# Farama-Foundation/HighwayEnv

Measured on NVIDIA H100. Metric: env-steps/sec (batched), highway-fast-v0 50 veh, higher is better.
Workload: dtype f64

## Files before the change

highwayenv_b200/csrc/hwy_highway.cu:

```cuda
#include <cstdio>
#include <cstdlib>
#include <cstring>
#include <algorithm>
#include <atomic>
#include <cstddef>
#include <mutex>

#include <cuda_runtime.h>

#include "../../include/hwyb200.h"
#include "hwy_device.cuh"
#include "hwy_math.cuh"

namespace hwy {

#ifdef HWY_PHASE_TIMING
__device__ unsigned long long g_phase_cycles[16];
#define PHASE_INIT() long long _pt = clock64()
#define PHASE_MARK(k)                                                                 \
    do {                                                                              \
        long long _n = clock64();                                                     \
        if ((threadIdx.x & 31) == 0) atomicAdd(&g_phase_cycles[k], (unsigned long long)(_n - _pt)); \
        _pt = _n;                                                                     \
    } while (0)
#else
#define PHASE_INIT()
#define PHASE_MARK(k)
#endif

template <int TPE>
struct Frame {
    static constexpr int NW = TPE / 32;
    double x[TPE], y[TPE], c[TPE], s[TPE], v[TPE], ts[TPE];
    double ls[TPE];
    __align__(16) float lsf[TPE];
    uint32_t smask[HWY_MAX_LANES][NW];
    uint32_t tm[HWY_MAX_LANES][NW];
    uint32_t lane_is[HWY_MAX_LANES][NW];
    uint32_t fired[NW];
    unsigned char lane[TPE], tgt[TPE], perm[TPE], rank[TPE];
    int slow;
    unsigned vmax_bits;
};

template <int TPE>
struct EnvShared {
    static constexpr int NW = TPE / 32;
    Frame<TPE> f[2];
    double key[TPE];
    uint32_t geo[TPE][NW];
    uint32_t mid[NW];
    uint32_t ok_left[NW], ok_right[NW];
    int n_items;
    unsigned short items[2 * TPE];
    double free_t[TPE], acc_own[TPE], delta[TPE];
    signed char f_own[TPE], r_own[TPE];
    uint32_t ctrl[NW], cc[NW];
    int last_will[TPE];
    unsigned char crash_hit[TPE];
    double sp_x[TPE];
    int done, sp_fallback;
};

template <int TPE>
__device__ __forceinline__ void env_sync() {
    __syncthreads();
}
template <int TPE, int LEVEL>
__device__ __forceinline__ void env_sync_phase() {
    __syncthreads();
}

template <int NW>
__device__ __forceinline__ bool test_bit(const uint32_t (&m)[NW], int i) {
    return (m[i >> 5] >> (i & 31)) & 1u;
}

__device__ __forceinline__ int lane_id() {
    int l;
    asm volatile("mov.u32 %0, %%laneid;" : "=r"(l));
    return l;
}

__device__ __forceinline__ void segment_or(uint32_t* words, uint32_t ballot, int i, int V) {
    const int lane = lane_id();
    if (i >= V || (i != 0 && lane != 0)) return;
    const int n = min(V - i, 32 - lane);
    const uint32_t m = (ballot >> lane) & (0xffffffffu >> (32 - n));
    if (!m) return;
    const int sh = i & 31;
    atomicOr(&words[i >> 5], m << sh);
    const uint32_t hi = __funnelshift_l(m, 0u, sh);
    if (hi) atomicOr(&words[(i >> 5) + 1], hi);
}
__device__ __forceinline__ uint32_t segment_leads(int i, bool active, int& mine) {
    const int lane = lane_id();
    const uint32_t lead = __ballot_sync(0xffffffffu, active && (i == 0 || lane == 0));
    mine = __popc(lead & (0xffffffffu >> (31 - lane))) - 1;
    return lead;
}

template <int TPE>
__device__ __noinline__ void neighbours_linear(const Frame<TPE>& F, const HwyStraightLane L, int V,
                                               int self, int& front, int& rear) {
    double s = lane_s(L, F.x[self], F.y[self]);
    double s_front = 0, s_rear = 0;
    front = -1;
    rear = -1;
    for (int v = 0; v < V; ++v) {
        if (v == self) continue;
        double s_v, lat_v;
        lane_local(L, F.x[v], F.y[v], s_v, lat_v);
        if (!lane_on(L, s_v, lat_v, 1.0)) continue;
        if (s <= s_v && (front < 0 || s_v <= s_front)) {
            s_front = s_v;
            front = v;
        }
        if (s_v < s && (rear < 0 || s_v > s_rear)) {
            s_rear = s_v;
            rear = v;
        }
    }
}

template <int TPE>
__device__ __forceinline__ void neighbours(const HwyHighwayParams& P, const Frame<TPE>& F, int V, int l,
                                           int self, int& front, int& rear) {
    constexpr int NW = TPE / 32;
    if (F.slow) {
        neighbours_linear(F, P.lanes[l], V, self, front, rear);
        return;
    }
    const int r = F.rank[self];
    const int w0 = r >> 5, b = r & 31;
    front = -1;
    rear = -1;
    uint32_t m = F.smask[l][w0] & (b == 31 ? 0u : (~0u << (b + 1)));
    int w = w0;
    while (m == 0 && ++w < NW) m = F.smask[l][w];
    if (m) front = F.perm[w * 32 + __ffs(m) - 1];
    m = F.smask[l][w0] & ((1u << b) - 1u);
    w = w0;
    while (m == 0 && --w >= 0) m = F.smask[l][w];
    if (m) rear = F.perm[w * 32 + 31 - __clz(m)];
}

template <int TPE>
__device__ __noinline__ int neighbours_packed(const uint32_t* __restrict__ smask_l, const Frame<TPE>& F, int self) {
    constexpr int NW = TPE / 32;
    const int r = F.rank[self];
    const int w0 = r >> 5, b = r & 31;
    int front = 0xff, rear = 0xff;
    uint32_t m = smask_l[w0] & (b == 31 ? 0u : (~0u << (b + 1)));
    int w = w0;
    while (m == 0 && ++w < NW) m = smask_l[w];
    if (m) front = F.perm[w * 32 + __ffs(m) - 1];
    m = smask_l[w0] & ((1u << b) - 1u);
    w = w0;
    while (m == 0 && --w >= 0) m = smask_l[w];
    if (m) rear = F.perm[w * 32 + 31 - __clz(m)];
    return front | (rear << 8);
}
template <int TPE>
__device__ __forceinline__ void neighbours_cold(const HwyHighwayParams& P, const Frame<TPE>& F, int V, int l,
                                                int self, int& front, int& rear) {
    if (F.slow) {
        neighbours_linear(F, P.lanes[l], V, self, front, rear);
        return;
    }
    const int fr = neighbours_packed(F.smask[l], F, self);
    front = (fr & 0xff) == 0xff ? -1 : (fr & 0xff);
    rear = (fr >> 8) == 0xff ? -1 : (fr >> 8);
}

struct IdmK {
    double comfort_acc_max, distance_wanted, time_wanted, two_sqrt_ab;
};
__device__ __forceinline__ IdmK make_idm(const HwyHighwayParams& P) {
    IdmK k;
    k.comfort_acc_max = P.comfort_acc_max;
    k.distance_wanted = P.distance_wanted;
    k.time_wanted = P.time_wanted;
    k.two_sqrt_ab = 2 * sqrt(-P.comfort_acc_max * P.comfort_acc_min);
    return k;
}
template <int TPE>
__device__ __forceinline__ double desired_gap(const IdmK& K, const Frame<TPE>& F, int ego, int front) {
    double dvx = F.v[ego] * F.c[ego] - F.v[front] * F.c[front];
    double dvy = F.v[ego] * F.s[ego] - F.v[front] * F.s[front];
    double dv = dot2(dvx, dvy, F.c[ego], F.s[ego]);
    return K.distance_wanted + F.v[ego] * K.time_wanted + F.v[ego] * dv / K.two_sqrt_ab;
}
template <int TPE>
__device__ __forceinline__ double lane_distance(const HwyHighwayParams& P, const Frame<TPE>& F,
                                                bool aligned, int ego, int other) {
// ... 186 lines not shown
                if (obs_env2) obs_env2[NF * pad + col] = 0.0f;
            }
        }
    } else if (i < K && i >= filled) {
        for (int col = 0; col < NF; ++col) {
            obs_env[NF * i + col] = 0.0f;
            if (obs_env2) obs_env2[NF * i + col] = 0.0f;
        }
    }
}

struct VehicleRegs {
    double x, y, heading, speed, target_speed, timer, delta, imp_x, imp_y;
    int meta;
};

__device__ __forceinline__ void load_vehicle(const HwyHighwayState& S, size_t slot, VehicleRegs& r) {
    double2 a = reinterpret_cast<const double2*>(S.pos)[slot];
    double2 b = reinterpret_cast<const double2*>(S.hs)[slot];
    double2 c = reinterpret_cast<const double2*>(S.tt)[slot];
    double2 d = reinterpret_cast<const double2*>(S.imp)[slot];
    r.x = a.x;
    r.y = a.y;
    r.heading = b.x;
    r.speed = b.y;
    r.target_speed = c.x;
    r.timer = c.y;
    r.imp_x = d.x;
    r.imp_y = d.y;
    r.delta = S.delta[slot];
    r.meta = S.meta[slot];
}
__device__ __forceinline__ void store_vehicle(const HwyHighwayState& S, size_t slot,
                                              const VehicleRegs& r) {
    reinterpret_cast<double2*>(S.pos)[slot] = make_double2(r.x, r.y);
    reinterpret_cast<double2*>(S.hs)[slot] = make_double2(r.heading, r.speed);
    reinterpret_cast<double2*>(S.tt)[slot] = make_double2(r.target_speed, r.timer);
    reinterpret_cast<double2*>(S.imp)[slot] = make_double2(r.imp_x, r.imp_y);
    S.meta[slot] = r.meta;
}

template <int TPE, bool LINEAR = false, bool DENSE = false>
__device__ __forceinline__ void publish(const HwyHighwayParams& P, Frame<TPE>& F, int i, bool active,
                                        const VehicleRegs& r) {
    constexpr int NW = TPE / 32;
    if (active) {
        double sn, cs;
        m_sincos(r.heading, &sn, &cs);
        F.x[i] = r.x;
        F.y[i] = r.y;
        F.c[i] = cs;
        F.s[i] = sn;
        F.v[i] = r.speed;
        F.ts[i] = meta_kind(r.meta) == HWY_KIND_VEHICLE ? (LINEAR ? r.speed : 0.0) : r.target_speed;
        F.ls[i] = lane_s(P.lanes[0], r.x, r.y);
        F.lsf[i] = (float)F.ls[i];
        F.lane[i] = (unsigned char)meta_lane(r.meta);
        F.tgt[i] = (unsigned char)meta_target(r.meta);
    }
    if (!DENSE && i < HWY_MAX_LANES * NW) (&F.smask[0][0])[i] = 0;
    if (i == 0) {
        F.slow = 0;
        F.vmax_bits = 0u;
    }
}

template <int TPE>
__device__ __forceinline__ void clear_masks(Frame<TPE>& F, int i, int V) {
    constexpr int kWords = (3 * HWY_MAX_LANES + 1) * (TPE / 32);
    static_assert(offsetof(Frame<TPE>, fired) + sizeof(F.fired) - offsetof(Frame<TPE>, smask) == 4 * kWords,
                  "mask words of Frame are not adjacent");
#pragma unroll 1
    for (int k = i; k < kWords; k += V) (&F.smask[0][0])[k] = 0;
}

template <int TPE>
__device__ __forceinline__ bool pair_precheck(const Frame<TPE>& F, int a, int b, double dt) {
    const double diag = sqrt(kVehLength * kVehLength + kVehWidth * kVehWidth);
    const double thr = (diag + diag) / 2 + F.v[a] * dt;
    const double dx = F.x[b] - F.x[a], dy = F.y[b] - F.y[a];
    return !(thr >= 0.0 && dx * dx + dy * dy > thr * thr * 1.000001 + 1e-9);
}
template <int TPE>
__device__ __noinline__ void pair_sat(const Frame<TPE>& F, int a, int b, double dt, bool& inter,
                                      bool& will, double& trx, double& try_) {
    {
        const double diag = sqrt(kVehLength * kVehLength + kVehWidth * kVehWidth);
        const double thr = (diag + diag) / 2 + F.v[a] * dt;
        const double dist = norm2(F.x[b] - F.x[a], F.y[b] - F.y[a]);
        if (dist > thr) {
            inter = false;
            will = false;
            trx = try_ = 0.0;
            return;
        }
    }
    {
        const double hl = kVehLength / 2, hw = kVehWidth / 2, margin = 1e-6;
        const double ca = F.c[a], sa = F.s[a], cb = F.c[b], sb = F.s[b];
        const double dx = F.x[b] - F.x[a], dy = F.y[b] - F.y[a];
        const double rvx = (F.v[a] * ca - F.v[b] * cb) * dt, rvy = (F.v[a] * sa - F.v[b] * sb) * dt;
        const double cd = fabs(ca * cb + sa * sb), sd = fabs(sa * cb - ca * sb);
        bool separated = false;
        separated |= fabs(dx * ca + dy * sa) - (hl + hl * cd + hw * sd) - fabs(rvx * ca + rvy * sa) > margin;
        separated |= fabs(-dx * sa + dy * ca) - (hw + hl * sd + hw * cd) - fabs(-rvx * sa + rvy * ca) > margin;
        separated |= fabs(dx * cb + dy * sb) - (hl + hl * cd + hw * sd) - fabs(rvx * cb + rvy * sb) > margin;
        separated |= fabs(-dx * sb + dy * cb) - (hw + hl * sd + hw * cd) - fabs(-rvx * sb + rvy * cb) > margin;
        if (separated) {
            inter = false;
            will = false;
            trx = try_ = 0.0;
            return;
        }
    }
    Quad pa = make_polygon(F.x[a], F.y[a], F.c[a], F.s[a]);
    Quad pb = make_polygon(F.x[b], F.y[b], F.c[b], F.s[b]);
    polygons_intersecting(pa, pb, F.v[a] * F.c[a] * dt, F.v[a] * F.s[a] * dt, F.v[b] * F.c[b] * dt,
                          F.v[b] * F.s[b] * dt, inter, will, trx, try_);
}

template <int TPE>
__device__ __noinline__ int rank_count(const Frame<TPE>& F, int V, int i, bool active) {
    const double si = active ? F.ls[i] : 0.0;
    const float fi = active ? F.lsf[i] : 0.0f;
    int rank = 0;
    bool ambiguous = false;
    const float4* lsf4 = reinterpret_cast<const float4*>(F.lsf);
    const int n4 = V >> 2;
    for (int q = 0; q < n4; ++q) {
        float4 f = lsf4[q];
        const int u = q << 2;
        rank += (f.x < fi) + (f.y < fi) + (f.z < fi) + (f.w < fi);
        ambiguous = ambiguous || (f.x == fi && u != i) || (f.y == fi && u + 1 != i) ||
                    (f.z == fi && u + 2 != i) || (f.w == fi && u + 3 != i);
    }
    for (int u = n4 << 2; u < V; ++u) {
        float fu = F.lsf[u];
        rank += fu < fi;
        ambiguous = ambiguous || (fu == fi && u != i);
    }
    bool tie = false;
    if (ambiguous) {
        rank = 0;
#pragma unroll 1
        for (int u = 0; u < V; ++u) {
            double su = F.ls[u];
            rank += (su < si) || (su == si && u < i);
            tie = tie || (su == si && u != i);
        }
    }
    return rank | ((int)tie << 8);
}

template <int TPE, bool DENSE>
__device__ __noinline__ int rank_repair(const Frame<TPE>& F, const Frame<TPE>& prev, int V, int i, bool active) {
    constexpr int NW = TPE / 32;
    uint32_t inv[NW];
    uint32_t bad = 0;
    if constexpr (!DENSE) {
        const int wl = i & 31;
#pragma unroll
        for (int w = 0; w < NW; ++w) {
            const int k = w * 32 + wl + 1;
            const bool in = k < V;
            const float a = in ? F.lsf[prev.perm[k - 1]] : 0.0f, c = in ? F.lsf[prev.perm[k]] : 1.0f;
            bool wrong = in && !(a < c) && !(a > c);
            if (in && a > c) {
                if (k >= 2 && !(F.lsf[prev.perm[k - 2]] < c)) wrong = true;
                if (k + 1 < V && !(a < F.lsf[prev.perm[k + 1]])) wrong = true;
            }
            inv[w] = __ballot_sync(0xffffffffu, in && a > c);
            bad |= __ballot_sync(0xffffffffu, wrong);
        }
    } else {
        const int lane = lane_id();
        int mine;
        int s = 0;
        for (uint32_t lead = segment_leads(i, active, mine); lead; lead &= lead - 1, ++s) {
            const ptrdiff_t d = (ptrdiff_t)(s - mine) * (ptrdiff_t)sizeof(EnvShared<TPE>);
            const Frame<TPE>& Fs = *reinterpret_cast<const Frame<TPE>*>(reinterpret_cast<const char*>(&F) + d);
            const Frame<TPE>& Ps = *reinterpret_cast<const Frame<TPE>*>(reinterpret_cast<const char*>(&prev) + d);
            uint32_t s_inv[NW];
            uint32_t s_bad = 0;
#pragma unroll
            for (int w = 0; w < NW; ++w) {
                const int k = w * 32 + lane + 1;
                const bool in = k < V;
                const float a = in ? Fs.lsf[Ps.perm[k - 1]] : 0.0f, c = in ? Fs.lsf[Ps.perm[k]] : 1.0f;
                bool wrong = in && !(a < c) && !(a > c);
                if (in && a > c) {
                    if (k >= 2 && !(Fs.lsf[Ps.perm[k - 2]] < c)) wrong = true;
                    if (k + 1 < V && !(a < Fs.lsf[Ps.perm[k + 1]])) wrong = true;
                }
                s_inv[w] = __ballot_sync(0xffffffffu, in && a > c);
                s_bad |= __ballot_sync(0xffffffffu, wrong);
            }
            if (s == mine) {
#pragma unroll
                for (int w = 0; w < NW; ++w) inv[w] = s_inv[w];
                bad = s_bad;
            }
        }
    }
#pragma unroll
    for (int w = 0; w < NW; ++w) {
        uint32_t near = (inv[w] << 1) | (inv[w] << 2);
        if (w > 0) near |= (inv[w - 1] >> 31) | (inv[w - 1] >> 30);
        bad |= inv[w] & near;
    }
    if (bad) return -1;
    if (!active) return 0;
    const int r0 = prev.rank[i];
    uint32_t w_dn = 0, w_up = 0;
#pragma unroll
    for (int w = 0; w < NW; ++w) {
        if (r0 >= 1 && w == ((r0 - 1) >> 5)) w_dn = inv[w];
        if (w == (r0 >> 5)) w_up = inv[w];
    }
    if (r0 >= 1 && ((w_dn >> ((r0 - 1) & 31)) & 1u)) return r0 - 1;
    if (r0 + 1 < V && ((w_up >> (r0 & 31)) & 1u)) return r0 + 1;
    return r0;
}

template <int TPE, bool DENSE>
__device__ __forceinline__ void build_frame(const HwyHighwayParams& P, EnvShared<TPE>& sm, Frame<TPE>& F,
                                            int i, bool active, bool aligned, const VehicleRegs& r,
                                            double dt, bool do_sweep, bool pruned, const Frame<TPE>* prev) {
    const int V = P.n_vehicles;
    const int wie = i >> 5;
    const int lane = meta_lane(r.meta), tgt = meta_target(r.meta);
    int rank = 0;
    bool reuse = false;
    if (prev && !DENSE) {
        bool ok = true;
#pragma unroll 1
        for (int k = (i & 31) + 1; k < V; k += 32) ok = ok && (F.lsf[prev->perm[k - 1]] < F.lsf[prev->perm[k]]);
        reuse = __all_sync(0xffffffffu, ok);
    } else if (prev) {
        int mine, s = 0;
#pragma unroll 1
        for (uint32_t lead = segment_leads(i, active, mine); lead; lead &= lead - 1, ++s) {
            const ptrdiff_t d = (ptrdiff_t)(s - mine) * (ptrdiff_t)sizeof(EnvShared<TPE>);
            const Frame<TPE>& Fs = *reinterpret_cast<const Frame<TPE>*>(reinterpret_cast<const char*>(&F) + d);
            const Frame<TPE>& Ps = *reinterpret_cast<const Frame<TPE>*>(reinterpret_cast<const char*>(prev) + d);
            bool ok = true;
#pragma unroll 1
            for (int k = lane_id() + 1; k < V; k += 32)
                ok = ok && (Fs.lsf[Ps.perm[k - 1]] < Fs.lsf[Ps.perm[k]]);
            ok = __all_sync(0xffffffffu, ok);
            if (s == mine) reuse = ok;
        }
    }
    bool tie = false;
    if constexpr (!DENSE) {
        if (reuse) {
            rank = active ? prev->rank[i] : 0;
        } else {
            int rt = (TPE >= 128 && prev) ? rank_repair<TPE, DENSE>(F, *prev, V, i, active) : -1;
            if (rt < 0) rt = rank_count(F, V, i, active);
            rank = rt & 0xff;
            tie = (rt >> 8) != 0;
        }
    } else {
        int rt = -1;
        if (TPE >= 128 && prev && __any_sync(0xffffffffu, !reuse)) rt = rank_repair<TPE, DENSE>(F, *prev, V, i, active);
        if (reuse) {
            rank = active ? prev->rank[i] : 0;
        } else if (active) {
            if (rt < 0) rt = rank_count(F, V, i, active);
            rank = rt & 0xff;
            tie = (rt >> 8) != 0;
        }
    }
    if (active) {
        F.perm[rank] = (unsigned char)i;
        F.rank[i] = (unsigned char)rank;
        if (tie || !aligned) F.slow = 1;
#pragma unroll 1
        for (int l = 0; l < P.lanes_count; ++l) {
            double s_l, lat_l;
            lane_local(P.lanes[l], r.x, r.y, s_l, lat_l);
            if (lane_on(P.lanes[l], s_l, lat_l, 1.0)) atomicOr(&F.smask[l][rank >> 5], 1u << (rank & 31));
        }
    }
    const bool is_idm = meta_kind(r.meta) == HWY_KIND_IDM;
#pragma unroll 1
    for (int l = 0; l < P.lanes_count; ++l) {
        uint32_t b_lane = __ballot_sync(0xffffffffu, active && lane == l);
        uint32_t b_tgt = __ballot_sync(0xffffffffu, active && tgt == l);
        if constexpr (DENSE) {
            segment_or(F.lane_is[l], b_lane, i, V);
            segment_or(F.tm[l], b_tgt, i, V);
        } else if ((i & 31) == 0) {
            F.lane_is[l][wie] = b_lane;
            F.tm[l][wie] = b_tgt;
        }
    }
    uint32_t b_fired = __ballot_sync(0xffffffffu, active && is_idm && lane == tgt && P.lane_change_delay < r.timer);
    if constexpr (DENSE)
        segment_or(F.fired, b_fired, i, V);
    else if ((i & 31) == 0)
        F.fired[wie] = b_fired;

    if (do_sweep && pruned) {
        if constexpr (DENSE) {
            if (active) {
                const int lane = lane_id(), lo = max(lane - i, 0), hi = min(lane - i + V, 32);
                const unsigned vb = __reduce_max_sync((0xffffffffu >> (32 - (hi - lo))) << lo,
                                                      __float_as_uint(fmaxf(__double2float_ru(r.speed), 0.0f)));
                if (lane == lo) atomicMax(&F.vmax_bits, vb);
            }
        } else {
            unsigned vb = __float_as_uint(active ? fmaxf(__double2float_ru(r.speed), 0.0f) : 0.0f);
            vb = __reduce_max_sync(0xffffffffu, vb);
            if ((i & 31) == 0) atomicMax(&F.vmax_bits, vb);
        }
    } else if (active && do_sweep) {
        const bool cc_i = test_bit(sm.cc, i);
        auto do_pair = [&](int a, int b) {
            if (!pair_precheck(F, a, b, dt)) return;
            bool inter, will;
            double trx, try_;
            pair_sat(F, a, b, dt, inter, will, trx, try_);
            if (will) {
                atomicMax(&sm.last_will[a], b);
                atomicMax(&sm.last_will[b], a);
            }
            if (inter) sm.crash_hit[a] = sm.crash_hit[b] = 1;
        };
#pragma unroll
        for (int w = 0; w < TPE / 32; ++w) {
            uint32_t m = sm.cc[w];
            if (w == (i >> 5)) m &= ~(1u << (i & 31));
            while (m) {
                int j = w * 32 + __ffs(m) - 1;
                m &= m - 1;
                if (cc_i) {
                    int k = j - i;
                    if (k < 0) k += V;
                    if (2 * k > V || (2 * k == V && i > j)) continue;
                }
                do_pair(i < j ? i : j, i < j ? j : i);
            }
        }
    }
}

template <int TPE>
__device__ __forceinline__ void sweep_pruned(EnvShared<TPE>& sm, const Frame<TPE>& F, int V, int i, bool active,
                                             double dt) {
    if (!active) return;
    const double diag = sqrt(kVehLength * kVehLength + kVehWidth * kVehWidth);
    const double bound = diag + (double)__uint_as_float(F.vmax_bits) * dt + 1e-6;
    const bool cc_i = test_bit(sm.cc, i);
    const double si = F.ls[i];
    for (int q = F.rank[i] + 1; q < V; ++q) {
        const int j = F.perm[q];
        if (F.ls[j] - si > bound) break;
        if (!(cc_i || test_bit(sm.cc, j))) continue;
        const int a = i < j ? i : j, b = i < j ? j : i;
        if (!pair_precheck(F, a, b, dt)) continue;
        bool inter, will;
        double trx, try_;
        pair_sat(F, a, b, dt, inter, will, trx, try_);
        if (will) {
            atomicMax(&sm.last_will[a], b);
            atomicMax(&sm.last_will[b], a);
        }
        if (inter) sm.crash_hit[a] = sm.crash_hit[b] = 1;
    }
}

template <int TPE>
__device__ __forceinline__ void apply_collisions(EnvShared<TPE>& sm, const Frame<TPE>& F, int i,
                                                 VehicleRegs& r, double dt) {
    if (sm.crash_hit[i]) {
        r.meta |= HWY_META_CRASHED;
        sm.crash_hit[i] = 0;
    }
    int j = sm.last_will[i];
    if (j >= 0) {
        int a = i < j ? i : j, b = i < j ? j : i;
        bool inter, will;
        double trx, try_;
        pair_sat(F, a, b, dt, inter, will, trx, try_);
        r.imp_x = i == a ? trx / 2 : -trx / 2;
        r.imp_y = i == a ? try_ / 2 : -try_ / 2;
        r.meta |= HWY_META_HAS_IMPACT;
        sm.last_will[i] = -1;
    }
}

constexpr int kPcgJumpN = 4 * HWY_MAX_VEHICLES + 8;
__device__ uint64_t g_pcg_jump[kPcgJumpN][4];

struct U128 {
    uint64_t hi, lo;
};
__device__ __forceinline__ U128 mul128(U128 a, U128 b) {
    U128 r;
    r.lo = a.lo * b.lo;
    r.hi = __umul64hi(a.lo, b.lo) + a.hi * b.lo + a.lo * b.hi;
    return r;
}
__device__ __forceinline__ U128 add128(U128 a, U128 b) {
    U128 r;
    r.lo = a.lo + b.lo;
    r.hi = a.hi + b.hi + (r.lo < a.lo ? 1 : 0);
    return r;
}
__device__ __forceinline__ Pcg64 pcg_at(const Pcg64& g0, int n) {
    U128 an = {g_pcg_jump[n][0], g_pcg_jump[n][1]}, gn = {g_pcg_jump[n][2], g_pcg_jump[n][3]};
    U128 st = add128(mul128(an, U128{g0.s_hi, g0.s_lo}), mul128(gn, U128{g0.i_hi, g0.i_lo}));
    Pcg64 g = g0;
    g.s_hi = st.hi;
    g.s_lo = st.lo;
    g.has32 = 0;
    g.u32 = 0;
    return g;
}
__device__ __forceinline__ Pcg64 pcg_at_far(const Pcg64& g0, int n) {
    Pcg64 g = g0;
    while (n >= kPcgJumpN) {
        g = pcg_at(g, kPcgJumpN - 1);
        n -= kPcgJumpN - 1;
// ... 473 lines not shown
    typedef unsigned __int128 u128;
    const u128 A = ((u128)0x2360ed051fc65da4ULL << 64) | 0x4385df649fccf645ULL;
    u128 an = 1, gn = 0;
    for (int n = 0; n < hwy::kPcgJumpN; ++n) {
        table[n][0] = (uint64_t)(an >> 64);
        table[n][1] = (uint64_t)an;
        table[n][2] = (uint64_t)(gn >> 64);
        table[n][3] = (uint64_t)gn;
        gn = gn * A + 1;
        an = an * A;
    }
    cudaError_t err = cudaMemcpyToSymbol(hwy::g_pcg_jump, table, sizeof(table));
    if (err != cudaSuccess) return fail("cudaMemcpyToSymbol(g_pcg_jump): %s", cudaGetErrorString(err));
    ready[dev] = true;
    return 0;
}

bool lanes_congruent_host(const HwyHighwayParams* p) {
    const HwyStraightLane* L = p->lanes;
    bool ok = L[0].dir_y == 0.0;
    for (int l = 1; l < p->lanes_count; ++l)
        ok = ok && L[l].start_x == L[0].start_x && L[l].dir_x == L[0].dir_x && L[l].dir_y == 0.0 &&
             L[l].heading == L[0].heading && L[l].length == L[0].length && L[l].lat_x == L[0].lat_x &&
             L[l].lat_y == L[0].lat_y;
    return ok;
}

template <int TPE, bool AL, bool DENSE>
int launch_step_kernel(const HwyHighwayParams* p, const HwyHighwayState* s, const HwyLinearTraffic* t,
                       const int32_t* action_i, const float* action_f, float* obs, double* reward,
                       uint8_t* terminated, uint8_t* truncated, double* info_speed, uint8_t* info_crashed,
                       int autoreset, float* final_obs, int epb, size_t env_bytes, int dev, cudaStream_t st) {
    const int blocks = (s->n_envs + epb - 1) / epb;
    const size_t smem = (size_t)epb * env_bytes;
    static std::atomic<size_t> configured[2][64];
    if (smem > configured[t != nullptr][dev].load(std::memory_order_relaxed)) {
        cudaError_t err = t ? cudaFuncSetAttribute(hwy::highway_linear_step_kernel<TPE, AL, DENSE>,
                                                   cudaFuncAttributeMaxDynamicSharedMemorySize, (int)smem)
                            : cudaFuncSetAttribute(hwy::highway_step_kernel<TPE, AL, DENSE>,
                                                   cudaFuncAttributeMaxDynamicSharedMemorySize, (int)smem);
        if (err != cudaSuccess) return fail("cudaFuncSetAttribute: %s", cudaGetErrorString(err));
        configured[t != nullptr][dev].store(smem, std::memory_order_relaxed);
    }
    const int threads = DENSE ? (epb * p->n_vehicles + 31) & ~31 : epb * TPE;
    if (t)
        hwy::highway_linear_step_kernel<TPE, AL, DENSE><<<blocks, threads, smem, st>>>(
            *p, *s, *t, action_i, action_f, obs, reward, terminated, truncated, info_speed, info_crashed,
            autoreset, final_obs, epb);
    else
        hwy::highway_step_kernel<TPE, AL, DENSE><<<blocks, threads, smem, st>>>(
            *p, *s, action_i, action_f, obs, reward, terminated, truncated, info_speed, info_crashed,
            autoreset, final_obs, epb);
    return 0;
}

template <int TPE, bool AL>
int launch_step(const HwyHighwayParams* p, const HwyHighwayState* s, const HwyLinearTraffic* t,
                const int32_t* action_i, const float* action_f, float* obs, double* reward, uint8_t* terminated,
                uint8_t* truncated, double* info_speed, uint8_t* info_crashed, int autoreset,
                float* final_obs, cudaStream_t st) {
    if (autoreset > 0 && ensure_pcg_jump(st)) return 1;
    int dev = 0;
    if (cudaGetDevice(&dev) != cudaSuccess || dev < 0 || dev >= 64) return fail("%s", "cudaGetDevice failed");
    const size_t env_bytes = sizeof(hwy::EnvShared<TPE>) + (t ? sizeof(hwy::LinearShared<TPE>) : 0);
    const int epb = step_envs_per_block(p->n_vehicles, env_bytes, s->n_envs, step_device(dev));
    const bool dense = epb * TPE > step_half_block_threads();
    if (dense)
        return launch_step_kernel<TPE, AL, true>(p, s, t, action_i, action_f, obs, reward, terminated, truncated,
                                                 info_speed, info_crashed, autoreset, final_obs, epb, env_bytes, dev,
                                                 st);
    return launch_step_kernel<TPE, AL, false>(p, s, t, action_i, action_f, obs, reward, terminated, truncated,
                                              info_speed, info_crashed, autoreset, final_obs, epb, env_bytes, dev, st);
}

int launch_observe(const HwyHighwayParams* p, const HwyHighwayState* s, const uint8_t* mask_a,
                   const uint8_t* mask_b, int use_mask, float* obs, cudaStream_t st) {
    int tpe = tpe_for(p->n_vehicles);
    Grid g = grid_for(tpe, s->n_envs);
    if (tpe == 32)
        hwy::highway_observe_kernel<32><<<g.blocks, g.threads, 0, st>>>(*p, *s, mask_a, mask_b, use_mask, obs);
    else if (tpe == 64)
        hwy::highway_observe_kernel<64><<<g.blocks, g.threads, 0, st>>>(*p, *s, mask_a, mask_b, use_mask, obs);
    else
        hwy::highway_observe_kernel<128><<<g.blocks, g.threads, 0, st>>>(*p, *s, mask_a, mask_b, use_mask, obs);
    return check_launch("highway_observe_kernel");
}

int launch_reset(const HwyHighwayParams* p, const HwyHighwayState* s, const uint8_t* mask_a,
                 const uint8_t* mask_b, int use_mask, cudaStream_t st) {
    int blocks = (s->n_envs + 127) / 128;
    hwy::highway_reset_kernel<<<blocks, 128, 0, st>>>(*p, *s, mask_a, mask_b, use_mask);
    return check_launch("highway_reset_kernel");
}

int launch_linear_reset(const HwyHighwayParams* p, const HwyHighwayState* s, const HwyLinearTraffic* t,
                        const uint8_t* mask_a, const uint8_t* mask_b, int use_mask, cudaStream_t st) {
    int blocks = (s->n_envs + 127) / 128;
    hwy::highway_linear_reset_kernel<<<blocks, 128, 0, st>>>(*p, *s, *t, mask_a, mask_b, use_mask);
    return check_launch("highway_linear_reset_kernel");
}

int validate_linear(const HwyLinearTraffic* t) {
    if (!t || !t->params) return fail("%s", "null linear traffic parameters");
    return 0;
}
}

namespace {
int dispatch_step(const HwyHighwayParams* p, const HwyHighwayState* s, const HwyLinearTraffic* t,
                  const int32_t* action_i, const float* action_f, float* obs, double* reward, uint8_t* terminated,
                  uint8_t* truncated, double* info_speed, uint8_t* info_crashed, int autoreset, float* final_obs,
                  cudaStream_t st);
int check_step_args(const HwyHighwayParams* p, const HwyHighwayState* s, const int32_t* action_i,
                    const float* action_f, float* obs, double* reward, uint8_t* terminated, uint8_t* truncated,
                    int autoreset);
}

extern "C" {

int hwy_abi_version(void) { return HWY_ABI_VERSION; }
const char* hwy_last_error(void) { return g_err; }
uint64_t hwy_launch_count(void) { return g_launches; }
int hwy_highway_slot_stride(int n_vehicles) { return (n_vehicles + 1) & ~1; }

int hwy_highway_observe(const HwyHighwayParams* p, const HwyHighwayState* s, float* obs, void* stream) {
    if (validate(p, s)) return 1;
    if (!obs) return fail("%s", "obs is null");
    return launch_observe(p, s, nullptr, nullptr, 0, obs, (cudaStream_t)stream);
}

int hwy_highway_reset(const HwyHighwayParams* p, const HwyHighwayState* s, const uint8_t* mask,
                      float* obs, void* stream) {
    if (validate(p, s)) return 1;
    cudaStream_t st = (cudaStream_t)stream;
    int use_mask = mask != nullptr;
    if (ensure_pcg_jump(st)) return 1;
    if (launch_reset(p, s, mask, nullptr, use_mask, st)) return 1;
    if (obs) return launch_observe(p, s, mask, nullptr, use_mask, obs, st);
    return 0;
}

int hwy_debug_phase_cycles(unsigned long long* out16) {
#ifdef HWY_PHASE_TIMING
    unsigned long long zero[16] = {0};
    if (cudaMemcpyFromSymbol(out16, hwy::g_phase_cycles, sizeof(zero)) != cudaSuccess) return 1;
    if (cudaMemcpyToSymbol(hwy::g_phase_cycles, zero, sizeof(zero)) != cudaSuccess) return 1;
    return 0;
#else
    for (int k = 0; k < 16; ++k) out16[k] = 0;
    return 0;
#endif
}

int hwy_debug_math(int op, const double* in, double* out, int n, void* stream) {
    if (op < HWY_MATH_SINCOS || op > HWY_MATH_SPEED_TO_INDEX) return fail("%s", "hwy_debug_math: unknown op");
    if (n < 0) return fail("%s", "hwy_debug_math: n < 0");
    if (!in || !out) return fail("%s", "hwy_debug_math: null pointer");
    if (n == 0) return 0;
    hwy::debug_math_kernel<<<(n + 127) / 128, 128, 0, (cudaStream_t)stream>>>(op, in, out, n);
    return check_launch("debug_math_kernel");
}

int hwy_debug_pcg64(int op, int arg_i, double arg_lo, double arg_hi, int count, const uint64_t* words_in,
                    uint64_t* words_out, uint64_t* draws, int n, void* stream) {
    if (op < HWY_PCG_NEXT64 || op > HWY_PCG_AT) return fail("%s", "hwy_debug_pcg64: unknown op");
    if (n < 0) return fail("%s", "hwy_debug_pcg64: n < 0");
    if (op == HWY_PCG_CHOICE && arg_i < 1) return fail("%s", "hwy_debug_pcg64: choice needs arg_i >= 1");
    if (op == HWY_PCG_AT && (arg_i < 0 || arg_i >= hwy::kPcgJumpN))
        return fail("%s", "hwy_debug_pcg64: pcg_at index outside the jump table");
    if (op != HWY_PCG_AT && (count < 0 || count > (1 << 20))) return fail("%s", "hwy_debug_pcg64: count outside 0..2^20");
    if (!words_in || !words_out || (op != HWY_PCG_AT && count > 0 && !draws))
        return fail("%s", "hwy_debug_pcg64: null pointer");
    if (n == 0) return 0;
    cudaStream_t st = (cudaStream_t)stream;
    if ((op == HWY_PCG_AT || op == HWY_PCG_NORMAL) && ensure_pcg_jump(st)) return 1;
    hwy::debug_pcg64_kernel<<<(n + 127) / 128, 128, 0, st>>>(op, arg_i, arg_lo, arg_hi, op == HWY_PCG_AT ? 0 : count,
                                                              words_in, words_out, draws, n);
    return check_launch("debug_pcg64_kernel");
}

int hwy_highway_autoreset(const HwyHighwayParams* p, const HwyHighwayState* s,
                          const uint8_t* terminated, const uint8_t* truncated, float* obs,
                          void* stream) {
    if (validate(p, s)) return 1;
    if (!terminated || !truncated || !obs) return fail("%s", "null pointer");
    cudaStream_t st = (cudaStream_t)stream;
    if (launch_reset(p, s, terminated, truncated, 1, st)) return 1;
    return launch_observe(p, s, terminated, truncated, 1, obs, st);
}

int hwy_highway_step(const HwyHighwayParams* p, const HwyHighwayState* s, const int32_t* action_i,
                     const float* action_f, float* obs, double* reward, uint8_t* terminated,
                     uint8_t* truncated, double* info_speed, uint8_t* info_crashed, int autoreset,
                     float* final_obs, void* stream) {
    if (check_step_args(p, s, action_i, action_f, obs, reward, terminated, truncated, autoreset)) return 1;
    return dispatch_step(p, s, nullptr, action_i, action_f, obs, reward, terminated, truncated, info_speed, info_crashed,
                         autoreset, final_obs, (cudaStream_t)stream);
}

int hwy_highway_substeps(const HwyHighwayParams* p, const HwyHighwayState* s, int n_substeps, const float* action_f,
                         void* stream) {
    if (validate(p, s)) return 1;
    if (n_substeps < 1 || n_substeps > 4096) return fail("%s", "n_substeps must be in 1..4096");
    return dispatch_step(p, s, nullptr, nullptr, action_f, nullptr, nullptr, nullptr, nullptr, nullptr, nullptr,
                         -n_substeps, nullptr, (cudaStream_t)stream);
}

int hwy_highway_linear_reset(const HwyHighwayParams* p, const HwyHighwayState* s, const HwyLinearTraffic* t,
                             const uint8_t* mask, float* obs, void* stream) {
    if (validate(p, s) || validate_linear(t)) return 1;
    cudaStream_t st = (cudaStream_t)stream;
    int use_mask = mask != nullptr;
    if (ensure_pcg_jump(st)) return 1;
    if (launch_linear_reset(p, s, t, mask, nullptr, use_mask, st)) return 1;
    if (obs) return launch_observe(p, s, mask, nullptr, use_mask, obs, st);
    return 0;
}

int hwy_highway_linear_autoreset(const HwyHighwayParams* p, const HwyHighwayState* s, const HwyLinearTraffic* t,
                                 const uint8_t* terminated, const uint8_t* truncated, float* obs, void* stream) {
    if (validate(p, s) || validate_linear(t)) return 1;
    if (!terminated || !truncated || !obs) return fail("%s", "null pointer");
    cudaStream_t st = (cudaStream_t)stream;
    if (launch_linear_reset(p, s, t, terminated, truncated, 1, st)) return 1;
    return launch_observe(p, s, terminated, truncated, 1, obs, st);
}

int hwy_highway_linear_step(const HwyHighwayParams* p, const HwyHighwayState* s, const HwyLinearTraffic* t,
                            const int32_t* action_i, const float* action_f, float* obs, double* reward,
                            uint8_t* terminated, uint8_t* truncated, double* info_speed, uint8_t* info_crashed,
                            int autoreset, float* final_obs, void* stream) {
    if (check_step_args(p, s, action_i, action_f, obs, reward, terminated, truncated, autoreset)) return 1;
    if (validate_linear(t)) return 1;
    return dispatch_step(p, s, t, action_i, action_f, obs, reward, terminated, truncated, info_speed, info_crashed,
                         autoreset, final_obs, (cudaStream_t)stream);
}

int hwy_highway_linear_substeps(const HwyHighwayParams* p, const HwyHighwayState* s, const HwyLinearTraffic* t,
                                int n_substeps, const float* action_f, void* stream) {
    if (validate(p, s) || validate_linear(t)) return 1;
    if (n_substeps < 1 || n_substeps > 4096) return fail("%s", "n_substeps must be in 1..4096");
    return dispatch_step(p, s, t, nullptr, action_f, nullptr, nullptr, nullptr, nullptr, nullptr, nullptr,
                         -n_substeps, nullptr, (cudaStream_t)stream);
}

}

namespace {
int check_step_args(const HwyHighwayParams* p, const HwyHighwayState* s, const int32_t* action_i,
                    const float* action_f, float* obs, double* reward, uint8_t* terminated, uint8_t* truncated,
                    int autoreset) {
    if (validate(p, s)) return 1;
    if (!obs || !reward || !terminated || !truncated) return fail("%s", "null output pointer");
    if (p->action_type == 0 && !action_i) return fail("%s", "DiscreteMetaAction needs action_i");
    if (p->action_type == 1 && !action_f) return fail("%s", "ContinuousAction needs action_f");
    if (autoreset != HWY_AUTORESET_DISABLED && autoreset != HWY_AUTORESET_SAME_STEP)
        return fail("%s", "unknown autoreset mode");
    return 0;
}

int dispatch_step(const HwyHighwayParams* p, const HwyHighwayState* s, const HwyLinearTraffic* t,
                  const int32_t* action_i, const float* action_f, float* obs, double* reward, uint8_t* terminated,
                  uint8_t* truncated, double* info_speed, uint8_t* info_crashed, int autoreset, float* final_obs,
                  cudaStream_t st) {
    int tpe = tpe_for(p->n_vehicles);
    const char* force_general = getenv("HWYB200_GENERAL_LANES");
    const bool al = lanes_congruent_host(p) && !(force_general && force_general[0] == '1');
#define HWY_LAUNCH_STEP(T, A)                                                                              \
    launch_step<T, A>(p, s, t, action_i, action_f, obs, reward, terminated, truncated, info_speed, info_crashed, \
                      autoreset, final_obs, st)
    int rc;
    if (tpe == 32)
        rc = al ? HWY_LAUNCH_STEP(32, true) : HWY_LAUNCH_STEP(32, false);
    else if (tpe == 64)
        rc = al ? HWY_LAUNCH_STEP(64, true) : HWY_LAUNCH_STEP(64, false);
    else
        rc = al ? HWY_LAUNCH_STEP(128, true) : HWY_LAUNCH_STEP(128, false);
#undef HWY_LAUNCH_STEP
    if (rc) return 1;
    if (check_launch(t ? "highway_linear_step_kernel" : "highway_step_kernel")) return 1;
    return 0;
}
}
```

highwayenv_b200/csrc/hwy_highway_step.cuh:

```cuda
    constexpr int NW = TPE / 32;
    extern __shared__ __align__(16) unsigned char smem_raw[];
    EnvShared<TPE>* smem = reinterpret_cast<EnvShared<TPE>*>(smem_raw);
    const int V = P.n_vehicles;
    const int EPB = DENSE ? dense_epb : blockDim.x / TPE;
    const int seg = threadIdx.x / (DENSE ? V : TPE);
    const int sub = DENSE && seg >= EPB ? EPB - 1 : seg;
    const int i = DENSE ? (seg < EPB ? threadIdx.x - seg * V : V) : threadIdx.x % TPE;
    const bool active = i < V;
    const int env = blockIdx.x * EPB + sub;
    const bool env_ok = (!DENSE || active) && env < S.n_envs;
    const int e = env < S.n_envs ? env : S.n_envs - 1;
    EnvShared<TPE>& sm = smem[sub];
    LinearShared<TPE>* lsm = nullptr;
    if constexpr (LINEAR) lsm = reinterpret_cast<LinearShared<TPE>*>(smem + EPB) + sub;
    const size_t slot = (size_t)e * S.vp + (active ? i : 0);
    const bool aligned = AL || lanes_aligned(P);
    const bool congruent = AL || lanes_congruent(P);

    VehicleRegs r;
    if constexpr (DENSE) {
        r = {};
        if (active) load_vehicle(S, slot, r);
    } else {
        load_vehicle(S, slot, r);
    }
    const int kind = meta_kind(r.meta);
    int speed_index = (i == 0) ? S.speed_index[e] : 0;
    double act_steer = 0.0, act_accel = 0.0;
    const int substeps_only = autoreset < 0 ? -autoreset : 0;
    const int frames = substeps_only ? substeps_only : P.simulation_frequency / P.policy_frequency;
    const double dt = 1.0 / P.simulation_frequency;

    {
        uint32_t b_cc = __ballot_sync(0xffffffffu, active && (r.meta & HWY_META_CHECK_COLLISIONS));
        uint32_t b_ctrl = __ballot_sync(0xffffffffu, active && kind != HWY_KIND_VEHICLE);
        if constexpr (DENSE) {
            if (i < NW) sm.cc[i] = sm.ctrl[i] = sm.mid[i] = 0;
            if (active) {
                sm.last_will[i] = -1;
                sm.crash_hit[i] = 0;
            }
        } else {
            if ((i & 31) == 0) {
                sm.cc[i >> 5] = b_cc;
                sm.ctrl[i >> 5] = b_ctrl;
                sm.mid[i >> 5] = 0;
            }
            sm.last_will[i] = -1;
            sm.crash_hit[i] = 0;
        }
        if (i < NW) sm.ok_left[i] = sm.ok_right[i] = 0;
        if (i == 0) sm.n_items = 0;
        if (active) sm.delta[i] = r.delta;
        if constexpr (LINEAR) {
            if (active) {
                const double* lp = T->params + slot * HWY_LINEAR_PARAMS;
                for (int k = 0; k < 3; ++k) lsm->acc[k][i] = lp[k];
                for (int k = 0; k < 2; ++k) lsm->steer[k][i] = lp[3 + k];
            }
        }
        if constexpr (DENSE) {
            __syncthreads();
            segment_or(sm.cc, b_cc, i, V);
            segment_or(sm.ctrl, b_ctrl, i, V);
        }
    }
    const IdmK K = make_idm(P);
    const bool pruned = P.others_check_collisions != 0;
    int p = 1;
    PHASE_INIT();
    PHASE_MARK(0);

    for (int frame = 0;; ++frame) {
        p ^= 1;
        Frame<TPE>& F = sm.f[p];
        publish<TPE, LINEAR, DENSE>(P, F, i, active, r);
        if (DENSE && active) clear_masks(F, i, V);
        PHASE_MARK(1);
        env_sync<TPE>();
        PHASE_MARK(2);
        if (i < NW) sm.mid[i] = sm.ok_left[i] = sm.ok_right[i] = 0;
        if (i == 0) sm.n_items = 0;
        build_frame<TPE, DENSE>(P, sm, F, i, active, aligned, r, dt, frame > 0, pruned,
                                frame > 0 ? &sm.f[p ^ 1] : nullptr);
        PHASE_MARK(3);
        if (pruned && frame > 0) {
            env_sync_phase<TPE, 3>();
            sweep_pruned(sm, F, V, i, active, dt);
        }
        env_sync_phase<TPE, 3>();
        PHASE_MARK(4);
        if (active && frame > 0) apply_collisions(sm, F, i, r, dt);
        PHASE_MARK(5);
        if (frame == frames) break;

        if (frame == 0) {
            if (i == 0) {
                if (kind == HWY_KIND_MDP) {
                    int a = substeps_only ? 1 : action_i[e];
                    if (a == 3 || a == 4) {
                        int idx = speed_to_index(P, r.speed) + (a == 3 ? 1 : -1);
                        idx = max(0, min(idx, P.n_target_speeds - 1));
                        speed_index = idx;
                        r.target_speed = P.target_speeds[idx];
                        F.ts[0] = r.target_speed;
                    } else if (a == 0 || a == 2) {
                        int old = meta_target(r.meta);
                        int id = old + (a == 2 ? 1 : -1);
                        id = max(0, min(id, P.lanes_count - 1));
                        if (lane_reachable(P.lanes[id], r.x, r.y)) {
                            r.meta = meta_set_target(r.meta, id);
                            F.tgt[0] = (unsigned char)id;
                            F.tm[old][0] &= ~1u;
                            F.tm[id][0] |= 1u;
                        }
                    }
                } else {
                    float a0 = action_f ? action_f[2 * (size_t)e] : 0.0f, a1 = action_f ? action_f[2 * (size_t)e + 1] : 0.0f;
                    if (P.act_clip) {
                        a0 = fminf(fmaxf(a0, -1.0f), 1.0f);
                        a1 = fminf(fmaxf(a1, -1.0f), 1.0f);
                    }
                    float acc = __fadd_rn((float)P.acc_lo,
                                          __fdiv_rn(__fmul_rn(__fsub_rn(a0, -1.0f),
                                                              (float)(P.acc_hi - P.acc_lo)), 2.0f));
                    float st = __fadd_rn((float)P.steer_lo,
                                         __fdiv_rn(__fmul_rn(__fsub_rn(a1, -1.0f),
                                                             (float)(P.steer_hi - P.steer_lo)), 2.0f));
                    act_accel = (double)acc;
                    act_steer = (double)st;
                }
            }
            env_sync<TPE>();
        }

        PHASE_MARK(6);
        const int lane = meta_lane(r.meta);
        const int tgt0 = meta_target(r.meta);
        const bool crashed = (r.meta & HWY_META_CRASHED) != 0;
        const bool idm_active = active && kind == HWY_KIND_IDM && !crashed;
        bool is_mid = false, fired = false;
        double acc = 0.0, free_i = 0.0;
        if (idm_active) {
            if constexpr (!LINEAR)
                free_i = idm_free_term(K.comfort_acc_max, r.speed, r.target_speed, P.lanes[lane].speed_limit, r.delta);
            int f_own, r_own;
            neighbours(P, F, V, lane, i, f_own, r_own);
            if constexpr (LINEAR) {
                acc = linear_acceleration(P, K, F, aligned, lsm->acc[0][i], lsm->acc[1][i], lsm->acc[2][i], i, f_own);
            } else {
                acc = free_i;
                if (f_own >= 0) acc -= idm_gap_term(P, K, F, aligned, i, f_own);
            }
            if (lane != tgt0) {
                is_mid = true;
                uint32_t g[NW];
#pragma unroll
                for (int w = 0; w < NW; ++w) {
                    uint32_t may = F.tm[tgt0][w];
                    uint32_t adj = (tgt0 > 0 ? F.lane_is[tgt0 - 1][w] : 0u) |
                                   (tgt0 < P.lanes_count - 1 ? F.lane_is[tgt0 + 1][w] : 0u);
                    may |= F.fired[w] & adj;
                    uint32_t cand = may & sm.ctrl[w] & ~F.lane_is[tgt0][w];
                    if (w == (i >> 5)) cand &= ~(1u << (i & 31));
                    g[w] = 0;
                    while (cand) {
                        int b = __ffs(cand) - 1;
                        cand &= cand - 1;
                        int v = w * 32 + b;
                        double d = lane_distance(P, F, aligned, i, v);
                        double d_star = desired_gap(K, F, i, v);
                        if (0 < d && d < d_star) g[w] |= 1u << b;
                    }
                    sm.geo[i][w] = g[w];
                }
                atomicOr(&sm.mid[i >> 5], 1u << (i & 31));
            } else if (P.lane_change_delay < r.timer) {
                r.timer = 0.0;
                fired = true;
                sm.free_t[i] = free_i;
                sm.acc_own[i] = acc;
                sm.f_own[i] = (signed char)f_own;
                sm.r_own[i] = (signed char)r_own;
                if (!(fabs(r.speed) < 1)) {
                    for (int k = 0; k < 2; ++k) {
                        int cand = k == 0 ? lane - 1 : lane + 1;
                        if (cand < 0 || cand > P.lanes_count - 1) continue;
                        if (!lane_reachable(P.lanes[cand], r.x, r.y)) continue;
                        int slot_ = atomicAdd(&sm.n_items, 1);
                        sm.items[slot_] = (unsigned short)(i | (cand << 8) | (k << 15));
                    }
                }
            }
        }
        PHASE_MARK(7);
        env_sync_phase<TPE, 2>();
        PHASE_MARK(8);

        if constexpr (LINEAR) {
            for (int t = i; (!DENSE || active) && t < sm.n_items; t += DENSE ? V : TPE) {
                const int it = sm.items[t];
                const int v = it & 0xff, cand = (it >> 8) & 0x7f, right = it >> 15;
                const double a0 = lsm->acc[0][v], a1 = lsm->acc[1][v], a2 = lsm->acc[2][v];
                int new_preceding, new_following;
                neighbours_cold(P, F, V, cand, v, new_preceding, new_following);
                double new_following_pred_a =
                    linear_acceleration(P, K, F, aligned, a0, a1, a2, new_following, v);
                if (new_following_pred_a < -P.lane_change_max_braking_imposed) continue;
                double self_pred_a = linear_acceleration(P, K, F, aligned, a0, a1, a2, v, new_preceding);
                double self_a = sm.acc_own[v];
                double jerk = self_pred_a - self_a;
                if (P.politeness != 0.0) {
                    const int f_o = sm.f_own[v], r_o = sm.r_own[v];
                    double new_following_a =
                        linear_acceleration(P, K, F, aligned, a0, a1, a2, new_following, new_preceding);
                    double old_following_a = linear_acceleration(P, K, F, aligned, a0, a1, a2, r_o, v);
                    double old_following_pred_a = linear_acceleration(P, K, F, aligned, a0, a1, a2, r_o, f_o);
                    jerk = self_pred_a - self_a +
                           P.politeness * (new_following_pred_a - new_following_a + old_following_pred_a -
                                           old_following_a);
                }
                if (jerk < P.lane_change_min_acc_gain) continue;
                atomicOr(right ? &sm.ok_right[v >> 5] : &sm.ok_left[v >> 5], 1u << (v & 31));
            }
        } else
        for (int t = i; (!DENSE || active) && t < sm.n_items; t += DENSE ? V : TPE) {
            const int it = sm.items[t];
            const int v = it & 0xff, cand = (it >> 8) & 0x7f, right = it >> 15;
            const double delta_v = sm.delta[v];
            int new_preceding, new_following;
            neighbours_cold(P, F, V, cand, v, new_preceding, new_following);
            double new_following_pred_a = idm_acceleration_of(P, K, F, aligned, delta_v, new_following, v);
            if (new_following_pred_a < -P.lane_change_max_braking_imposed) continue;
            double self_pred_a = sm.free_t[v];
            if (new_preceding >= 0) self_pred_a -= idm_gap_term(P, K, F, aligned, v, new_preceding);
// ... 198 lines not shown
```

Measured before the change: 12.21 million.

## Rank vehicles by bounded local search using per-frame max longitudinal shift

For 64-thread-per-env configurations, each frame publishes the warp/segment-wide maximum forward and backward longitudinal displacement. Each vehicle then recomputes its rank by scanning only the neighbours in the previous order that could have crossed it. The O(V) rank count, and the reuse/repair checks, are only needed as a fallback when ties appear. This adds atomics, a reset of the shift maxima, and an early-exit loop that is data dependent. Debug tallies of which rank path was taken are compiled in only under phase timing.

```diff
diff --git a/highwayenv_b200/csrc/hwy_highway.cu b/highwayenv_b200/csrc/hwy_highway.cu
--- a/highwayenv_b200/csrc/hwy_highway.cu
+++ b/highwayenv_b200/csrc/hwy_highway.cu
@@ -16,6 +16,7 @@
 
 #ifdef HWY_PHASE_TIMING
 __device__ unsigned long long g_phase_cycles[16];
+__device__ unsigned long long g_rank_paths[8];
 #define PHASE_INIT() long long _pt = clock64()
 #define PHASE_MARK(k)                                                                 \
     do {                                                                              \
@@ -23,9 +24,15 @@
         if ((threadIdx.x & 31) == 0) atomicAdd(&g_phase_cycles[k], (unsigned long long)(_n - _pt)); \
         _pt = _n;                                                                     \
     } while (0)
+#define RANK_TALLY(k, cond)                                                           \
+    do {                                                                              \
+        const unsigned _b = __ballot_sync(0xffffffffu, (cond));                       \
+        if ((threadIdx.x & 31) == 0 && _b) atomicAdd(&g_rank_paths[k], (unsigned long long)__popc(_b)); \
+    } while (0)
 #else
 #define PHASE_INIT()
 #define PHASE_MARK(k)
+#define RANK_TALLY(k, cond)
 #endif
 
 template <int TPE>
@@ -41,6 +48,7 @@
     unsigned char lane[TPE], tgt[TPE], perm[TPE], rank[TPE];
     int slow;
     unsigned vmax_bits;
+    unsigned shift_fwd, shift_back;
 };
 
 template <int TPE>
@@ -533,6 +541,64 @@
     return rank | ((int)tie << 8);
 }
 
+__device__ __forceinline__ unsigned order_bits(float f) {
+    const unsigned b = __float_as_uint(f);
+    return b ^ ((b >> 31) ? 0xffffffffu : 0x80000000u);
+}
+__device__ __forceinline__ float order_float(unsigned o) { return __uint_as_float(o ^ ((o >> 31) ? 0x80000000u : 0xffffffffu)); }
+
+template <int TPE, bool DENSE>
+__device__ __forceinline__ void publish_shift(Frame<TPE>& F, const Frame<TPE>& prev, int i, bool active, int V) {
+    const double d = active ? F.ls[i] - prev.ls[i] : 0.0;
+    unsigned fwd = active ? order_bits(__double2float_ru(d)) : 0u;
+    unsigned back = active ? order_bits(__double2float_ru(-d)) : 0u;
+    if constexpr (DENSE) {
+        if (active) {
+            const int lane = lane_id(), lo = max(lane - i, 0), hi = min(lane - i + V, 32);
+            const unsigned m = (0xffffffffu >> (32 - (hi - lo))) << lo;
+            fwd = __reduce_max_sync(m, fwd);
+            back = __reduce_max_sync(m, back);
+            if (lane == lo) {
+                atomicMax(&F.shift_fwd, fwd);
+                atomicMax(&F.shift_back, back);
+            }
+        }
+    } else {
+        fwd = __reduce_max_sync(0xffffffffu, fwd);
+        back = __reduce_max_sync(0xffffffffu, back);
+        if ((i & 31) == 0) {
+            atomicMax(&F.shift_fwd, fwd);
+            atomicMax(&F.shift_back, back);
+        }
+    }
+}
+
+template <int TPE>
+__device__ __forceinline__ int rank_shift(const Frame<TPE>& F, const Frame<TPE>& prev, int V, int i, double fwd,
+                                          double back) {
+    const int r0 = prev.rank[i];
+    const double si = prev.ls[i], ni = F.ls[i], di = ni - si;
+    const double up = di + back + 1e-6, down = fwd - di + 1e-6;
+    int rank = r0;
+#pragma unroll 1
+    for (int k = r0 + 1; k < V; ++k) {
+        const int u = prev.perm[k];
+        if (prev.ls[u] - si > up) break;
+        const double nu = F.ls[u];
+        if (nu == ni) return -1;
+        rank += nu < ni;
+    }
+#pragma unroll 1
+    for (int k = r0 - 1; k >= 0; --k) {
+        const int u = prev.perm[k];
+        if (si - prev.ls[u] > down) break;
+        const double nu = F.ls[u];
+        if (nu == ni) return -1;
+        rank -= nu > ni;
+    }
+    return rank;
+}
+
 template <int TPE, bool DENSE>
 __device__ __noinline__ int rank_repair(const Frame<TPE>& F, const Frame<TPE>& prev, int V, int i, bool active) {
     constexpr int NW = TPE / 32;
@@ -611,47 +677,78 @@
     const int wie = i >> 5;
     const int lane = meta_lane(r.meta), tgt = meta_target(r.meta);
     int rank = 0;
-    bool reuse = false;
-    if (prev && !DENSE) {
-        bool ok = true;
-#pragma unroll 1
-        for (int k = (i & 31) + 1; k < V; k += 32) ok = ok && (F.lsf[prev->perm[k - 1]] < F.lsf[prev->perm[k]]);
-        reuse = __all_sync(0xffffffffu, ok);
-    } else if (prev) {
-        int mine, s = 0;
-#pragma unroll 1
-        for (uint32_t lead = segment_leads(i, active, mine); lead; lead &= lead - 1, ++s) {
-            const ptrdiff_t d = (ptrdiff_t)(s - mine) * (ptrdiff_t)sizeof(EnvShared<TPE>);
-            const Frame<TPE>& Fs = *reinterpret_cast<const Frame<TPE>*>(reinterpret_cast<const char*>(&F) + d);
-            const Frame<TPE>& Ps = *reinterpret_cast<const Frame<TPE>*>(reinterpret_cast<const char*>(prev) + d);
-            bool ok = true;
-#pragma unroll 1
-            for (int k = lane_id() + 1; k < V; k += 32)
-                ok = ok && (Fs.lsf[Ps.perm[k - 1]] < Fs.lsf[Ps.perm[k]]);
-            ok = __all_sync(0xffffffffu, ok);
-            if (s == mine) reuse = ok;
-        }
-    }
     bool tie = false;
-    if constexpr (!DENSE) {
-        if (reuse) {
-            rank = active ? prev->rank[i] : 0;
-        } else {
-            int rt = (TPE >= 128 && prev) ? rank_repair<TPE, DENSE>(F, *prev, V, i, active) : -1;
+    [[maybe_unused]] int path = 0;
+    if constexpr (TPE == 64) {
+        if (active) {
+            int rt = -1;
+            if (prev) {
+                const float fwd = order_float(F.shift_fwd), back = order_float(F.shift_back);
+                if (isfinite(fwd) && isfinite(back)) rt = rank_shift(F, *prev, V, i, (double)fwd, (double)back);
+                path = rt < 0 ? 3 : rt == prev->rank[i] ? 1 : 2;
+            }
             if (rt < 0) rt = rank_count(F, V, i, active);
             rank = rt & 0xff;
             tie = (rt >> 8) != 0;
         }
     } else {
-        int rt = -1;
-        if (TPE >= 128 && prev && __any_sync(0xffffffffu, !reuse)) rt = rank_repair<TPE, DENSE>(F, *prev, V, i, active);
-        if (reuse) {
-            rank = active ? prev->rank[i] : 0;
-        } else if (active) {
-            if (rt < 0) rt = rank_count(F, V, i, active);
-            rank = rt & 0xff;
-            tie = (rt >> 8) != 0;
-        }
+        bool reuse = false;
+        if (prev && !DENSE) {
+            bool ok = true;
+#pragma unroll 1
+            for (int k = (i & 31) + 1; k < V; k += 32) ok = ok && (F.lsf[prev->perm[k - 1]] < F.lsf[prev->perm[k]]);
+            reuse = __all_sync(0xffffffffu, ok);
+        } else if (prev) {
+            int mine, s = 0;
+#pragma unroll 1
+            for (uint32_t lead = segment_leads(i, active, mine); lead; lead &= lead - 1, ++s) {
+                const ptrdiff_t d = (ptrdiff_t)(s - mine) * (ptrdiff_t)sizeof(EnvShared<TPE>);
+                const Frame<TPE>& Fs = *reinterpret_cast<const Frame<TPE>*>(reinterpret_cast<const char*>(&F) + d);
+                const Frame<TPE>& Ps = *reinterpret_cast<const Frame<TPE>*>(reinterpret_cast<const char*>(prev) + d);
+                bool ok = true;
+#pragma unroll 1
+                for (int k = lane_id() + 1; k < V; k += 32)
+                    ok = ok && (Fs.lsf[Ps.perm[k - 1]] < Fs.lsf[Ps.perm[k]]);
+                ok = __all_sync(0xffffffffu, ok);
+                if (s == mine) reuse = ok;
+            }
+        }
+        path = 1;
+        if constexpr (!DENSE) {
+            if (reuse) {
+                rank = active ? prev->rank[i] : 0;
+            } else {
+                int rt = (TPE >= 128 && prev) ? rank_repair<TPE, DENSE>(F, *prev, V, i, active) : -1;
+                path = 2;
+                if (rt < 0) {
+                    rt = rank_count(F, V, i, active);
+                    path = 3;
+                }
+                rank = rt & 0xff;
+                tie = (rt >> 8) != 0;
+            }
+        } else {
+            int rt = -1;
+            if (TPE >= 128 && prev && __any_sync(0xffffffffu, !reuse)) rt = rank_repair<TPE, DENSE>(F, *prev, V, i, active);
+            if (reuse) {
+                rank = active ? prev->rank[i] : 0;
+            } else if (active) {
+                path = 2;
+                if (rt < 0) {
+                    rt = rank_count(F, V, i, active);
+                    path = 3;
+                }
+                rank = rt & 0xff;
+                tie = (rt >> 8) != 0;
+            }
+        }
+    }
+    if (prev) {
+        RANK_TALLY(0, active);
+        RANK_TALLY(1, active && path == 1);
+        RANK_TALLY(2, active && path == 2);
+        RANK_TALLY(3, active && path == 3);
+        RANK_TALLY(4, active && tie);
     }
     if (active) {
         F.perm[rank] = (unsigned char)i;
@@ -1431,6 +1528,15 @@
 #endif
 }
 
+#ifdef HWY_PHASE_TIMING
+int hwy_debug_rank_paths(unsigned long long* out8) {
+    unsigned long long zero[8] = {0};
+    if (cudaMemcpyFromSymbol(out8, hwy::g_rank_paths, sizeof(zero)) != cudaSuccess) return 1;
+    if (cudaMemcpyToSymbol(hwy::g_rank_paths, zero, sizeof(zero)) != cudaSuccess) return 1;
+    return 0;
+}
+#endif
+
 int hwy_debug_math(int op, const double* in, double* out, int n, void* stream) {
     if (op < HWY_MATH_SINCOS || op > HWY_MATH_SPEED_TO_INDEX) return fail("%s", "hwy_debug_math: unknown op");
     if (n < 0) return fail("%s", "hwy_debug_math: n < 0");
diff --git a/highwayenv_b200/csrc/hwy_highway_step.cuh b/highwayenv_b200/csrc/hwy_highway_step.cuh
--- a/highwayenv_b200/csrc/hwy_highway_step.cuh
+++ b/highwayenv_b200/csrc/hwy_highway_step.cuh
@@ -75,12 +75,16 @@
         p ^= 1;
         Frame<TPE>& F = sm.f[p];
         publish<TPE, LINEAR, DENSE>(P, F, i, active, r);
+        if (TPE == 64 && frame > 0) publish_shift<TPE, DENSE>(F, sm.f[p ^ 1], i, active, V);
         if (DENSE && active) clear_masks(F, i, V);
         PHASE_MARK(1);
         env_sync<TPE>();
         PHASE_MARK(2);
         if (i < NW) sm.mid[i] = sm.ok_left[i] = sm.ok_right[i] = 0;
-        if (i == 0) sm.n_items = 0;
+        if (i == 0) {
+            sm.n_items = 0;
+            sm.f[p ^ 1].shift_fwd = sm.f[p ^ 1].shift_back = 0u;
+        }
         build_frame<TPE, DENSE>(P, sm, F, i, active, aligned, r, dt, frame > 0, pruned,
                                 frame > 0 ? &sm.f[p ^ 1] : nullptr);
         PHASE_MARK(3);
```

Result: faster. 12.51 million, median of 6 (+2.4%).
